# yl602019618/Reconstruction-of-PDE-without-Time-Label

Measured on AMD Instinct MI355X. Metric: snapshot-bags/sec (train step) + rel-L2 drift error, 2D FPE 128² @1/2/4/8 GPU, higher is better.
Workload: dtype f32; 1 GPU; 2d_FPE train_fno.py NIOFP2D_FNO(2,3,100,25,3,12,32,2) (C), grid 128x128; per_gpu_batch=4, global_batch=4, T=100, bag_size=L=randint(50,T) with replacement, dataset_bags=4096, parallelism=dp1, optimizer=Adam lr 0.0005 (fused flat), launch=hip-graph per bag size L (all kernels replayed each step)

## Files before the change

### include/blindno.h

```cpp
#ifndef BLINDNO_H
#define BLINDNO_H

#include <stdint.h>

#ifdef __cplusplus
extern "C" {
#endif

typedef void* blindno_stream_t;

int blindno_abi_version(void);
const char* blindno_error_string(int code);


int blindno_lift_fwd(const float* in, const float* w0, const float* b0, float* x0,
                     int Bn, int N1, int N2, int Cin, int C, int P1, int P2,
                     blindno_stream_t stream);

int blindno_lift_bwd(const float* dx0, const float* in, const float* w0, float* d_in,
                     float* partial, int nchunk,
                     int Bn, int N1, int N2, int Cin, int C, int P1, int P2,
                     blindno_stream_t stream);
int blindno_lift_bwd_nchunk(int Bn, int N1, int N2);

int blindno_project_fwd(const float* z, const float* w1, const float* b1, const float* w2,
                        const float* b2, float* out, int Bn, int C, int P1, int P2, int Ho,
                        int Wo, int Hd, int Cout, int ostride, int ooff,
                        blindno_stream_t stream);

int blindno_project_bwd(const float* z, const float* w1, const float* b1, const float* w2,
                        const float* dout, float* dz, float* partial, int nchunk,
                        int Bn, int C, int P1, int P2, int Ho, int Wo, int Hd, int Cout,
                        int ostride, int ooff, int dout_div, blindno_stream_t stream);
int blindno_project_bwd_nchunk(int Bn, int Ho, int Wo);
int blindno_project_bwd_nchunk_heads(int Bg, int Ho, int Wo);
int blindno_project_bwd_w(const float* z, const float* w1, const float* b1, const float* w2,
                          const float* dout, const float* lscale, float* dz, float* partial,
                          int nchunk, int Bn, int C, int P1, int P2, int Ho, int Wo, int Hd,
                          int Cout, int ostride, int ooff, int dout_div, blindno_stream_t stream);

int64_t blindno_project_bag_stats_floats(int B, int Ho, int Wo);
int blindno_project_bag_bwd_nchunk(int B, int Ho, int Wo);
int blindno_project_bag_fwd(const float* z, const float* w1, const float* b1, const float* w2,
                            const float* b2, const float* lw, float* ubar, float* stats,
                            float* v, int B, int U, int C, int P1, int P2, int Ho, int Wo, int Hd,
                            blindno_stream_t stream);
int blindno_project_bag_bwd(const float* stats, const float* gs, const float* w2, const float* lw,
                            const float* v, float* dz, float* partial, int nchunk, int B, int U,
                            int C, int P1, int P2, int Ho, int Wo, int Hd,
                            blindno_stream_t stream);


int blindno_rowdft(const float* x, float* At, const float* Tp, int Bn, int C, int P1,
                   int P2, int m2, int act, blindno_stream_t stream);
int blindno_rowdft_crop(const float* x, float* At, const float* Tp, int Bn, int C, int P1,
                        int P2, int m2, int act, int N1v, int N2v, blindno_stream_t stream);

int blindno_colpass(const float* At, const float* Wt, float* Xs, float* Y, float* Z,
                    const float* FB, const float* GB, int Bn, int Ci, int Co, int P1, int m1,
                    int m2, int P2, int dir, blindno_stream_t stream);

int blindno_mix_wgrad_nsplit(int Bn, int Ci, int Co, int K1, int m2);
int blindno_mix_wgrad(const float* X, const float* G, float* dWt, float* partial, int nsplit,
                      int Bn, int Ci, int Co, int K1, int m2, blindno_stream_t stream);
int blindno_mix_wgrad_part(const float* X, const float* G, float* partial, int nsplit, int Gw,
                           int Bn, int Ci, int Co, int K1, int m2, blindno_stream_t stream);
int blindno_mix_wgrad_multi(const void* const* X, const void* const* G, void* const* out,
                            const int* shp, int njobs, blindno_stream_t stream);
int blindno_mix_wgrad_multi_u(const void* const* X, const void* const* G, void* const* out,
                              const int* shp, void* const* ud, const int* um1, int njobs,
                              blindno_stream_t stream);

int blindno_mix1d(const float* At, const float* Wt, float* Xs, float* Z, int Bn, int Ci,
                  int Co, int m, int P2, int dir, blindno_stream_t stream);

int blindno_rowidft_epi(const float* Z, const float* x, const float* wc, const float* bc,
                        float* z, const float* tb, int Bn, int C, int P1, int P2, int m2,
                        int act, blindno_stream_t stream);
int blindno_rowidft_epi_crop(const float* Z, const float* x, const float* wc, const float* bc,
// ... 385 lines not shown
```

### reconstruction-of-pde-without-time-label_amd/blindno/_lib.py

```python
from __future__ import annotations

import ctypes
import os
import threading

import torch

_HERE = os.path.dirname(os.path.abspath(__file__))
LIB_PATH = os.environ.get("BLINDNO_LIB", os.path.join(_HERE, "libblindno.so"))

SIGNATURES = {
    "blindno_abi_version": "",
    "blindno_lift_fwd": "ppppiiiiiiis",
    "blindno_lift_bwd": "pppppiiiiiiiis",
    "blindno_project_fwd": "ppppppiiiiiiiiiis",
    "blindno_project_bwd": "pppppppiiiiiiiiiiiis",
    "blindno_rowdft": "pppiiiiiis",
    "blindno_rowdft_crop": "pppiiiiiiiis",
    "blindno_rowdft_bag_lift": "ppppppiiiiiiiiis",
    "blindno_rowdft_bag_lift_dg": "pppppppiiiiiiiiis",
    "blindno_rowidft_epi_lift": "ppppppppppiiiiiiiiis",
    "blindno_rowidft_bwd_lift": "ppppppppppiiiiiiiiis",
    "blindno_colpass": "pppppppiiiiiiiis",
    "blindno_colspec_ok": "iiiiii",
# ... 36 lines not shown
    "blindno_mse_fwd": "ppplipppps",
    "blindno_rowsq": "pppiiiiiis",
    "blindno_adam": "pppplddffffs",
    "blindno_gpe_solve": "ppppddiiipppiiis",
    "blindno_trapz_rows": "ppppiis",
    "blindno_lift_bwd_nchunk": "iii",
    "blindno_conv_wgrad_nchunk": "iii",
    "blindno_rowidft_bwd_nchunk": "iiiii",
    "blindno_set_rowfuse": "i",
    "blindno_set_colfuse": "i",
    "blindno_project_bwd_nchunk": "iii",
    "blindno_project_bwd_nchunk_heads": "iii",
    "blindno_mix_wgrad_nsplit": "iiiii",
    "blindno_lift_fwd_g": "ppppiliiiiiiis",
    "blindno_lift_fwd_bag_g": "ppppiliiiiiiippppfs",
    "blindno_lift_bag_ok": "iiiiiiii",
    "blindno_lift_bwd_g": "pppppiiliiiiiiis",
    "blindno_lift_bwd_mix_g": "pppppiiliiiiiiippppiiis",
    "blindno_lift_bwd_bag_mix_g": "pppppiiliiiiiiippppiiippppffs",
    "blindno_project_fwd_g": "ppppppiliiiiiiiiiis",
    "blindno_project_bwd_g": "pppppppiiliiiiiiiiiis",
    "blindno_colpass_g": "pppppppiliiiiiiiis",
    "blindno_mix_wgrad_g": "ppppiiiiiiis",
    "blindno_rowidft_epi_g": "ppppppiliiiiiis",
    "blindno_rowidft_bwd_g": "ppppppiliiiiiis",
    "blindno_conv_wgrad_g": "pppiiiiiiis",
    "blindno_rowdft_wgrad_ok": "iiiii",
    "blindno_rowdft_wgrad_g": "pppppiippppiiiiiiiis",
    "blindno_bagmean_fwd_w": "pppppp" + "iiiii" + "s",
    "blindno_project_bwd_w": "pppppppp" + "i" + "iiiiiiiiiii" + "s",
    "blindno_project_bag_stats_floats": "iii",
    "blindno_project_bag_bwd_nchunk": "iii",
    "blindno_project_bag_fwd": "ppppppppp" + "iiiiiiii" + "s",
    "blindno_project_bag_bwd": "ppppppp" + "i" + "iiiiiiii" + "s",
    "blindno_pack_w2d_2": "ppppp" + "iiiii" + "s",
    "blindno_unpack_w2d_2": "ppppp" + "iiiii" + "s",
    "blindno_bn_act_nslices": "iii",
    "blindno_bn_act_fwd": "ppppppppiiiifffis",
    "blindno_bn_act_bwd": "pppppppppiiiifis",
    "blindno_gather_flat": "pppips",
    "blindno_gather_batch": "ppppipis",
    "blindno_reduce_partials_multi": "ppppis",
    "blindno_reduce_partials_pieces": "ppppppis",
    "blindno_reduce_partials_pieces_u": "pppppppppis",
    "blindno_reduce_segs_limit": "i",
    "blindno_finish_multi": "pppppppppippppis",
    "blindno_unpack_w2d_multi": "ppppis",
    "blindno_pack_w2d_multi": "ppppis",
    "blindno_fp_propagate": "pppiiiiiids",
    "blindno_bagattn_nchunk": "i",
    "blindno_bagattn_fwd": "pppppppp" + "iiii" + "s",
    "blindno_bagattn_bwd": "ppppppppppp" + "iiii" + "s",
    "blindno_conv2d_fwd": "pppp" + "iiiiiiiiiii" + "s",
    "blindno_conv2d_bwd_data": "ppp" + "iiiiiiiiiii" + "s",
    "blindno_conv2d_wgrad_nsplit": "iiiiiiiiiii",
    "blindno_conv2d_bwd_weight": "pppp" + "i" + "iiiiiiiiiii" + "s",
    "blindno_conv2d_fwd_nsplit": "iiiiiiiiiii",
    "blindno_conv2d_fwd_split": "ppppp" + "i" + "p" + "iiiiiiiiiii" + "s",
    "blindno_conv2d_bwd_data_nsplit": "iiiiiiiiiii",
    "blindno_conv2d_bwd_data_split": "pppp" + "i" + "p" + "iiiiiiiiiii" + "s",
    "blindno_conv2d_wscratch_floats": "i" + "iiiiiiiiiii",
    "blindno_spectral2d_tables_bytes": "iiii",
    "blindno_spectral2d_tables_init": "piiii",
    "blindno_spectral_conv2d_workspace_bytes": "iiiiiiii",
    "blindno_spectral_conv2d_saved_bytes": "iiiii",
    "blindno_spectral_conv2d_fwd": "ppppppp" + "iiiiiii" + "s",
# ... 129 lines not shown
```

### reconstruction-of-pde-without-time-label_amd/blindno/ops.py

```python
from __future__ import annotations

import contextlib
import ctypes
import math
from typing import List, Optional, Sequence, Tuple

import torch

from ._lib import BlindnoError, call, ptr, query, stream_ptr

F32 = torch.float32

MIX_F16 = False

BAG_STATS = True
BAG_STATS_MAX_BYTES = 4 << 30

COLSPEC = True
HEAD_BWD_MERGED = True
UNPACK_FOLD = True
HOST_ENC_MIX = True
HOST_PACK = True


def set_mix_precision(name: str) -> None:
    global MIX_F16
    if name not in ("fp32", "fp16"):
        raise BlindnoError(f"mix precision must be 'fp32' or 'fp16', got {name!r}")
    MIX_F16 = name == "fp16"


def _mixdir(direction: int) -> int:
    return direction | (2 if MIX_F16 else 0)



def pad_amount(n: int) -> int:
    return int(round(n * 0.25))


def kept_rows_count(m1: int, P1: int) -> int:
    return 2 * m1 if 2 * m1 < P1 else P1


_TW = {}


def twiddle(P: int, device) -> torch.Tensor:
    dev = torch.device(device)
# ... 1373 lines not shown
         ptr(twiddle_colspec(P1, m1, grid.device)), 1, 3, P1, P2, m2, 0, P1, P2, stream_ptr())
    K1 = kept_rows_count(m1, P1)
    Dg2 = _empty(1, m2, 3, K1, 2, like=grid)
    call("blindno_colmix", ptr(part), nb, None, ptr(Dg2), None, 1, 3, 3, P1, P2, m1, m2, 0, None, None,
         None, stream_ptr())
    if not capturing:
        if len(_DG2_CACHE) > 16:
            _DG2_CACHE.clear()
        _DG2_CACHE[key] = (grid, Dg2)
    return Dg2


class _ColSpec:

    def __init__(self, Bn, C, P1, P2, m1, m2, device):
        self.Bn, self.C, self.P1, self.P2, self.m1, self.m2 = Bn, C, P1, P2, m1, m2
        self.K1 = kept_rows_count(m1, P1)
        self.nb = P1 // 16
        self.tab = twiddle_colspec(P1, m1, device)
        self.Tp = twiddle_mfma(P2, m2, device)
        self.tb = twiddle_rowinv(P2, m2, device)

    def part(self, Cp, like):
        return _empty(self.Bn * self.nb * query("blindno_colspec_nchunk", Cp, self.m2) * 128, like=like)

    def mix(self, part, nbv, Wt, direction, Cp=None, lift=None):
        Xs = _empty(self.Bn, self.m2, self.C, self.K1, 2, like=part)
        Y = _empty(self.Bn, self.m2, self.C, self.K1, 2, like=part)
        w0, b0, Dg2 = lift if lift is not None else (None, None, None)
        call("blindno_colmix", ptr(part), nbv, ptr(Wt), ptr(Xs), ptr(Y), self.Bn, self.C,
             Cp or self.C, self.P1, self.P2, self.m1, self.m2, direction, ptr(w0), ptr(b0), ptr(Dg2),
             stream_ptr())
        return Xs, Y


def _bag_stats_ok(B, L, C, P1, P2, Ho, Wo, Hd, Cout):
    if not (BAG_STATS and Hd == 128 and Cout == 1 and L <= 1024):
        return False
    nstats = query("blindno_project_bag_stats_floats", B, Ho, Wo)
    return 4 * (nstats + B * L * C * P1 * P2) <= BAG_STATS_MAX_BYTES


def bag_ubar_ok(meta, B, L, N1, N2, fc1w, fc2w, head_meta, G, width):
    fake = (B * L, N1, N2, 3)
    _, _, _, _, P1, P2, Ho, Wo = _fno_geometry(fake, meta)
    if not _bag_stats_ok(B, L, meta.width, P1, P2, Ho, Wo, fc1w.shape[0], fc2w.shape[0]):
        return False
    hP1, hP2 = _fno_geometry((B, N1, N2, width), head_meta)[4:6]
    return query("blindno_lift_bag_ok", G, G * B, N1, N2, width, head_meta.width, hP1, hP2) == 1


class BagHeadsIn:

    def __init__(self, grid, bw, bb):
        self.grid, self.w, self.b = _c(grid), _c(bw.detach()), _c(bb.detach())
        self.width = bw.shape[0]

    def shape(self, ubar):
        return (ubar.shape[0], ubar.shape[1], ubar.shape[2], self.width)


class BagEncoderFn(torch.autograd.Function):

    @staticmethod
    def forward(ctx, meta, emit_ubar, X, idx_t, lw, grid, bw, bb, *prm):
        require_device(X, grid, *prm)
# ... 65 lines not shown
                tb = ptr(twiddle_rowinv(P2, meta.m2, X.device))
                if last:
                    call("blindno_rowidft_epi_lift", ptr(Z), ptr(X), ptr(idx_t), ptr(grid), ptr(fc0w),
                         ptr(fc0b), ptr(cw), ptr(cb), ptr(z), tb, B, T, L, N1, N2, C, P1, P2,
                         meta.m2, stream_ptr())
                else:
                    At_next = _empty(Bn, meta.m2, C, P1, 2, like=X)
                    call("blindno_rowidft_epi_lift_rd", ptr(Z), ptr(X), ptr(idx_t), ptr(grid),
                         ptr(fc0w), ptr(fc0b), ptr(cw), ptr(cb), ptr(z), tb, B, T, L, N1, N2, C, P1,
                         P2, meta.m2, ptr(At_next), ptr(twiddle_mfma(P2, meta.m2, X.device)), 1,
                         stream_ptr())
            else:
                Xk, Z = spec_forward(zs[-1], 1, Wt, sh, At=At_next)
                if last:
                    z = _empty(Bn, C, P1, P2, like=X)
                    call("blindno_rowidft_epi_crop", ptr(Z), ptr(zs[-1]), ptr(cw), ptr(cb), ptr(z),
                         ptr(twiddle_rowinv(P2, meta.m2, X.device)), Bn, C, P1, P2, meta.m2, 1, Ho, Wo,
                         stream_ptr())
                else:
                    z, At_next = k_rowidft_epi_rd(Z, zs[-1], cw, cb, Bn, C, P1, P2, meta.m2, 1, 1)
            Xs.append(Xk)
            Wts.append(Wt)
            zs.append(z)
        fc1w, fc1b, fc2w, fc2b = prm[2 + 4 * n:6 + 4 * n]
        Hd, Cout = fc1w.shape[0], fc2w.shape[0]
        S = Ho * Wo
        width = bw.shape[0]
        h = _empty(B, S, width, like=X)
        ctx.bag = None
        if _bag_stats_ok(B, L, C, P1, P2, Ho, Wo, Hd, Cout):
            ubar = _empty(B, S, like=X)
            stats = _empty(query("blindno_project_bag_stats_floats", B, Ho, Wo), like=X)
            v = _empty(Bn, C, P1, P2, like=X)
            call("blindno_project_bag_fwd", ptr(zs[-1]), ptr(fc1w), ptr(fc1b), ptr(fc2w), ptr(fc2b),
                 ptr(lw), ptr(ubar), ptr(stats), ptr(v), B, L, C, P1, P2, Ho, Wo, Hd, stream_ptr())
            if not emit_ubar:
                call("blindno_bagmean_fwd_w", ptr(ubar), ptr(grid), ptr(bw), ptr(bb), None, ptr(h), B, 1,
                     S, 2, width, stream_ptr())
            ctx.bag = (stats, v)
        elif emit_ubar:
            raise BlindnoError("BagEncoderFn: emit_ubar needs the bag-level projection (bag_ubar_ok)")
        else:
            u = _empty(Bn, Ho, Wo, Cout, like=X)
            call("blindno_project_fwd", ptr(zs[-1]), ptr(fc1w), ptr(fc1b), ptr(fc2w), ptr(fc2b), ptr(u),
                 Bn, C, P1, P2, Ho, Wo, Hd, Cout, Cout, 0, stream_ptr())
            call("blindno_bagmean_fwd_w", ptr(u), ptr(grid), ptr(bw), ptr(bb), ptr(lw), ptr(h), B, L, S,
                 2, width, stream_ptr())
        ctx.meta, ctx.n, ctx.dims = meta, n, (B, T, L, N1, N2, C, P1, P2, Ho, Wo, Hd, Cout, width)
        ctx.lw = lw
        ctx.emit_ubar = bool(emit_ubar)
        ctx.save_for_backward(X, idx_t, grid, bw, *Xs, *Wts, *zs, *prm)
        if emit_ubar:
            return ubar.view(B, N1, N2)
        return h.view(B, N1, N2, width)

    @staticmethod
    def backward(ctx, gh):
        meta, n = ctx.meta, ctx.n
        B, T, L, N1, N2, C, P1, P2, Ho, Wo, Hd, Cout, width = ctx.dims
        t = ctx.saved_tensors
        X, idx_t, grid, bw = t[:4]
        Xs, Wts, zs = list(t[4:4 + n]), list(t[4 + n:4 + 2 * n]), list(t[4 + 2 * n:4 + 3 * n])
        prm = list(t[4 + 3 * n:])
        Bn, S = B * L, Ho * Wo
        gh = _c(gh)
        grads = [None] * len(prm)
        lw = ctx.lw
        bag = ctx.bag
# ... 510 lines not shown
```

### reconstruction-of-pde-without-time-label_amd/blindno/timing.py

```python
from __future__ import annotations

import os

import torch

from . import _lib

GELU_FLOPS = 0
DOMINANT = os.environ.get("BLINDNO_TIMED_KERNEL", "blindno_project_bag_fwd")
_VARIANTS = {"blindno_project_bwd": ("blindno_project_bwd", "blindno_project_bwd_w"),
             "blindno_conv2d": ("blindno_conv2d_fwd", "blindno_conv2d_bwd_data", "blindno_conv2d_bwd_weight",
                                "blindno_conv2d_fwd_split", "blindno_conv2d_bwd_data_split")}
_CONV_ARG0 = {"blindno_conv2d_fwd": 4, "blindno_conv2d_bwd_data": 3, "blindno_conv2d_bwd_weight": 5,
              "blindno_conv2d_fwd_split": 7, "blindno_conv2d_bwd_data_split": 6}
_FAMILIES = ("blindno_conv2d",)


def _conv_out(n, k, s, p):
    return (n + 2 * p - k) // s + 1


def _i(args, k):
    return int(args[k])


def _present(a):
    return a is not None and getattr(a, "value", a) is not None


def cost(name, args):
    if name == "blindno_rowdft":
        Bn, C, P1, P2, m2 = (_i(args, k) for k in range(3, 8))
        return 4 * Bn * C * P1 * P2 + 8 * Bn * m2 * C * P1, 4 * Bn * C * P1 * P2 * m2
    if name == "blindno_rowidft_epi":
        has_wc = _present(args[2])
        Bn, C, P1, P2, m2 = (_i(args, k) for k in range(6, 11))
        pts = Bn * C * P1 * P2
        return 8 * Bn * C * P1 * m2 + 4 * pts * (2 if has_wc else 1), pts * (4 * m2 + (2 * C if has_wc else 0))
    if name == "blindno_rowidft_bwd":
        has_wc, act = _present(args[2]), _i(args, 11)
        Bn, C, P1, P2, m2 = (_i(args, k) for k in range(6, 11))
        pts = Bn * C * P1 * P2
        return (8 * Bn * C * P1 * m2 + 4 * pts * (2 + int(has_wc) + int(act > 0)),
                pts * (4 * m2 + (2 * C if has_wc else 0)))
    if name == "blindno_project_fwd":
        Bn, C, P1, P2, Ho, Wo, Hd, Cout = (_i(args, k) for k in range(6, 14))
        pts = Bn * Ho * Wo
        return 4 * pts * (C + Cout), pts * Hd * (2 * C + 2 * Cout + GELU_FLOPS)
    if name in ("blindno_project_bwd", "blindno_project_bwd_w"):
        o = 8 if name == "blindno_project_bwd" else 9
        Bn, C, P1, P2, Ho, Wo, Hd, Cout = (_i(args, k) for k in range(o, o + 8))
        dout_div = _i(args, o + 10)
        pts = Bn * Ho * Wo
        return (8 * pts * C + 4 * (pts // max(1, dout_div)) * Cout,
                pts * Hd * (6 * C + 4 * Cout + 1 + 2 * GELU_FLOPS))
    if name == "blindno_project_bag_fwd":
        B, U, C, P1, P2, Ho, Wo, Hd = (_i(args, k) for k in range(9, 17))
        pts, bpts = B * U * Ho * Wo, B * Ho * Wo
        return (8 * pts * C + 4 * ((bpts + 15) // 16) * 16 * Hd * 6 + 4 * bpts,
                pts * Hd * (6 * C + 4 + 2 * GELU_FLOPS))
    if name == "blindno_project_bag_bwd":
        B, U, C, P1, P2, Ho, Wo, Hd = (_i(args, k) for k in range(8, 16))
        pts, bpts = B * U * Ho * Wo, B * Ho * Wo
        return 8 * pts * C + 4 * ((bpts + 15) // 16) * 16 * Hd * 6 + 4 * bpts, 2 * bpts * Hd * 6
    if name in _CONV_ARG0:
        o = _CONV_ARG0[name]
        N, Ci, Hi, Wi, Co, KH, KW, sh, sw, ph, pw = (_i(args, k) for k in range(o, o + 11))
        Ho, Wo = _conv_out(Hi, KH, sh, ph), _conv_out(Wi, KW, sw, pw)
        K = Ci * KH * KW + (1 if name == "blindno_conv2d_bwd_weight" else 0)
        flops = 2 * N * Co * Ho * Wo * K
        nbytes = 4 * (N * Ci * Hi * Wi + N * Co * Ho * Wo + Co * K)
        return nbytes, flops
    if name == "blindno_colpass3d":
        Bn, Ci, Co, P1, P2, P3, m1, m2, m3, d = (_i(args, k) for k in range(7, 17))
        cin, cout = (Ci, Co) if d == 0 else (Co, Ci)
        K1, K2 = min(2 * m1, P1), min(2 * m2, P2)
        nbytes = 8 * (Bn * m3 * (cin + cout) * P1 * P2 + Bn * m3 * cin * K1 * K2 + m3 * K1 * K2 * Ci * Co)
        flops = 8 * Bn * m3 * ((cin + cout) * (P1 * P2 * K2 + P1 * K2 * K1) + K1 * K2 * Ci * Co)
        return nbytes, flops
    if name == "blindno_conv_wgrad":
        nchunk, Bn, C, P1, P2 = (_i(args, k) for k in range(3, 8))
        pts = Bn * P1 * P2
        return 8 * C * pts, 2 * pts * (C * C + C)
    return 0, 0


def pmc_record(root: str, name: str):
    import json
    p = os.path.join(root, "profiles", "pmc_traffic.json")
    if not os.path.exists(p):
        return None
    return json.load(open(p)).get(name)


def pmc_traffic(root: str, name: str):
    import json
    p = os.path.join(root, "profiles", "pmc_traffic.json")
    if not os.path.exists(p):
        return None
    d = json.load(open(p)).get(name)
    return None if d is None else float(d["bytes_per_point"])


def points(name, args):
    if name == "blindno_project_bag_fwd":
        return _i(args, 9) * _i(args, 10) * _i(args, 14) * _i(args, 15)
    if name in ("blindno_project_bwd", "blindno_project_bwd_w", "blindno_project_fwd"):
        o = {"blindno_project_bwd": 8, "blindno_project_bwd_w": 9, "blindno_project_fwd": 6}[name]
        Bn, Ho, Wo = _i(args, o), _i(args, o + 4), _i(args, o + 5)
        return Bn * Ho * Wo
    return 0


class KernelTimer:

    def __init__(self, name: str = DOMINANT):
        self.name = name
        self.entries = _VARIANTS.get(name, (name,))
        self.recs = []
        self._pending = None

    class _Hook:
        def __init__(self, timer, entry):
            self.timer, self.entry = timer, entry

        def before(self, args):
            ev = torch.cuda.Event(enable_timing=True)
            ev.record()
            self.timer._pending = ev

        def after(self, args):
            ev = torch.cuda.Event(enable_timing=True)
            ev.record()
            b, f = cost(self.entry, args)
            self.timer.recs.append((self.timer._pending, ev, b, f, points(self.entry, args)))

    def start(self):
        for e in self.entries:
# ... 45 lines not shown
```

### reconstruction-of-pde-without-time-label_amd/build.py

```python
#!/usr/bin/env python3
from __future__ import annotations

import argparse
import concurrent.futures as cf
import glob
import os
import shutil
import subprocess
import sys

HERE = os.path.dirname(os.path.abspath(__file__))
CSRC = os.path.join(HERE, "csrc")
OUT = os.path.join(HERE, "blindno", "libblindno.so")
BUILD = os.path.join(HERE, "build")
INCLUDE = os.path.join(os.path.dirname(HERE), "include")
ARCH = os.environ.get("BLINDNO_ARCH", "gfx950")

CXXFLAGS = ["-O3", "-fPIC", "-std=c++17", f"--offload-arch={ARCH}", "-I", INCLUDE, "-I", CSRC,
            "-fvisibility=hidden", "-Wall", "-Wno-unused-function", "-Wno-unused-result"]


FILE_FLAGS = {"project.hip": ["-fno-slp-vectorize", "-mllvm", "-amdgpu-mfma-vgpr-form"],
              "bagproj.hip": ["-fno-slp-vectorize", "-mllvm", "-amdgpu-mfma-vgpr-form"]}


def _hipcc():
    h = shutil.which("hipcc") or "/opt/rocm/bin/hipcc"
    if not os.path.exists(h):
        raise RuntimeError("hipcc not found (ROCm toolchain required to build libblindno)")
    return h


def _newer(src_list, dst):
    if not os.path.exists(dst):
        return True
    t = os.path.getmtime(dst)
    return any(os.path.getmtime(s) > t for s in src_list)


def build(force: bool = False, jobs: int = 8, verbose: bool = True) -> str:
    hipcc = _hipcc()
    os.makedirs(BUILD, exist_ok=True)
    srcs = sorted(glob.glob(os.path.join(CSRC, "*.hip")))
    headers = glob.glob(os.path.join(CSRC, "*.h")) + glob.glob(os.path.join(INCLUDE, "*.h"))
    objs = []
    todo = []
    for s in srcs:
        o = os.path.join(BUILD, os.path.basename(s)[:-4] + ".o")
        objs.append(o)
        if force or _newer([s] + headers, o):
            todo.append((s, o))

    def compile_one(so):
        s, o = so
        cmd = [hipcc, *CXXFLAGS, *FILE_FLAGS.get(os.path.basename(s), []), "-c", s, "-o", o]
        r = subprocess.run(cmd, capture_output=True, text=True)
# ... 48 lines not shown
```

### reconstruction-of-pde-without-time-label_amd/csrc/bagproj.hip

```cpp
#include "common.h"
#include "blindno.h"
#include "gelu_pk.h"

using namespace blindno;
using namespace blindno::gelu_pk;

namespace {

typedef float f32x4 __attribute__((ext_vector_type(4)));

constexpr int kHd = 128;
constexpr int kNStat = 6;
constexpr int kTileF4 = (kHd / 16) * kNStat * 64;
constexpr int kMaxU = 1024;
#ifndef BAGPROJ_QUAD
#define BAGPROJ_QUAD 1
#endif
#ifndef BAGPROJ_FWD_WAVES
#define BAGPROJ_FWD_WAVES 3
#endif
#ifndef BAGPROJ_SETUP2
#define BAGPROJ_SETUP2 1
#endif

// ... 11 lines not shown
#define BAGPROJ_BWD_UNROLL 1
#endif
#ifndef BAGPROJ_SC
#define BAGPROJ_SC 8
#endif
constexpr int kSC2 = BAGPROJ_SC;

__device__ __forceinline__ float swap_sum32(float a, float b) {
  const auto r = __builtin_amdgcn_permlane32_swap(__float_as_uint(a), __float_as_uint(b), false, false);
  return __uint_as_float(r[0]) + __uint_as_float(r[1]);
}

__device__ __forceinline__ float swap_sum16(float a, float b) {
  const auto r = __builtin_amdgcn_permlane16_swap(__float_as_uint(a), __float_as_uint(b), false, false);
  return __uint_as_float(r[0]) + __uint_as_float(r[1]);
}

#ifndef BAGPROJ_PROBE
#define BAGPROJ_PROBE 0
#endif
#if BAGPROJ_PROBE
__device__ unsigned long long g_bagproj_probe[32768 * 8];
#define BP_MARK(i)                                                                          \
  do {                                                                                      \
    __builtin_amdgcn_sched_barrier(0);                                                      \
    const unsigned long long t_ = __builtin_amdgcn_s_memrealtime();                         \
    const int slot_ = blockIdx.x * 4 + (threadIdx.x >> 6);                                  \
    if ((threadIdx.x & 63) == 0 && slot_ < 32768) g_bagproj_probe[slot_ * 8 + (i)] = t_;    \
    __builtin_amdgcn_sched_barrier(0);                                                      \
  } while (0)
#else
#define BP_MARK(i) do {} while (0)
#endif
__global__ __launch_bounds__(256, BAGPROJ_FWD_WAVES) void bagproj_fwd_kernel(
    const float* __restrict__ z, const float* __restrict__ w1, const float* __restrict__ b1,
    const float* __restrict__ w2, const float* __restrict__ b2, const float* __restrict__ lw,
    float* __restrict__ ubar, float* __restrict__ stats, float* __restrict__ v, BagGeom g) {
  __shared__ float slw[kMaxU];
  __shared__ float zs[2][kSC2][16][4];
  __shared__ float zw[2][kSC2][16][4];
  __shared__ float vred[2][4][kSC2][64];
  __shared__ float zbr[4][64];
  __shared__ float vpart[16][4];
  __shared__ float vhalf[4];
  __shared__ float ured[4][16];
  __shared__ float2 swr[4][4][2][2][4];
  const int tid = threadIdx.x, lane = tid & 63;
  const int wave = uniform_int(tid >> 6);
  const int c16 = lane & 15, g4 = lane >> 4;
  const int C = (int)g.C, U = (int)g.U;
  BP_MARK(0);
  const int cs = (tid >> 4) & 3, ls = tid >> 6;
  const unsigned ntiles = (g.npts + 15) / 16;
  auto zload = [&](unsigned bo, bool ok, int ch, float (&zr)[kSC2 / 4]) {
#pragma unroll
    for (int i = 0; i < kSC2 / 4; ++i) {
      const int lg = ch * kSC2 + ls + 4 * i;
#if BAGPROJ_SETUP2
      const int lc = lg < U ? lg : U - 1, cc = cs < C ? cs : C - 1;
      const float zv = z[bo + (unsigned)(lc * C + cc) * g.HW];
      zr[i] = (ok && lg < U && cs < C) ? zv : 0.f;
#else
      zr[i] = (ok && lg < U && cs < C) ? z[bo + (unsigned)(lg * C + cs) * g.HW] : 0.f;
#endif
    }
  };
  float wa[2], bb[2][4], vloc[4] = {0.f, 0.f, 0.f, 0.f};
#if BAGPROJ_SETUP2
  __shared__ float sw1[kHd * 4], sb1[kHd], sw2[kHd];
  constexpr int kLwIt = kMaxU / 256;
  float lwv[kLwIt], w1v[2], b1v = 0.f, w2v = 0.f;
#pragma unroll
  for (int i = 0; i < kLwIt; ++i) {
    const int l = tid + 256 * i;
    lwv[i] = l < U ? (lw ? lw[l] : 1.0f / (float)U) : 0.f;
  }
#pragma unroll
  for (int i = 0; i < 2; ++i) w1v[i] = tid + 256 * i < kHd * C ? w1[tid + 256 * i] : 0.f;
  if (tid < kHd) {
    b1v = b1[tid];
    w2v = w2[tid];
  }
  float zfirst[kSC2 / 4];
  {
    const unsigned f = blockIdx.x * 16 + (unsigned)c16;
    const bool ok = f < g.npts;
    zload(g.base(ok ? f : 0u), ok, 0, zfirst);
  }
#pragma unroll
  for (int i = 0; i < kLwIt; ++i)
    if (tid + 256 * i < U) slw[tid + 256 * i] = lwv[i];
#pragma unroll
  for (int i = 0; i < 2; ++i)
    if (tid + 256 * i < kHd * C) sw1[tid + 256 * i] = w1v[i];
// ... 32 lines not shown
    for (int r = 0; r < 4; ++r) {
      const int k = k0 + 4 * g4 + r;
      bb[tt][r] = kK * b1[k];
      if (c16 == 0) {
#pragma unroll
        for (int c = 0; c < 4; ++c) {
          const float wrv = c < C ? w2[k] * w1[k * C + c] : 0.f;
          vloc[c] += wrv;
          float2& e = swr[wave][g4][tt][r >> 1][c];
          if (r & 1) e.y = wrv; else e.x = wrv;
        }
      }
    }
  }
#endif
  if (c16 == 0) {
#pragma unroll
    for (int c = 0; c < 4; ++c) vpart[4 * wave + g4][c] = 0.5f * vloc[c];
  }
  __syncthreads();
  if (tid < 4) {
    float acc = 0.f;
    for (int j = 0; j < 16; ++j) acc += vpart[j][tid];
    vhalf[tid] = acc;
  }
#if !BAGPROJ_SETUP2
  float lsum = 0.f;
  for (int l = 0; l < U; ++l) lsum += slw[l];
  const float b2l = b2[0] * lsum;
#endif
  BP_MARK(1);

  const int nch = (U + kSC2 - 1) / kSC2;
  for (unsigned tile = blockIdx.x; tile < ntiles; tile += gridDim.x) {
    const unsigned f = tile * 16 + (unsigned)c16;
    const bool ok = f < g.npts;
    const unsigned bo = g.base(ok ? f : 0u);
    float zbp = 0.f;
    float zn[kSC2 / 4];
    auto load = [&](int ch) { zload(bo, ok, ch, zn); };
    auto store = [&](int ch, int buf) {
#pragma unroll
      for (int i = 0; i < kSC2 / 4; ++i) {
        const int l = ls + 4 * i, lg = ch * kSC2 + l;
        const float wv = zn[i] * slw[lg < U ? lg : 0];
        zs[buf][l][c16][cs] = zn[i];
        zw[buf][l][c16][cs] = wv;
        zbp += wv;
      }
    };
    auto vwrite = [&](int ch, int buf) {
#pragma unroll
      for (int i = 0; i < kSC2 / 4; ++i) {
        const int l = ls + 4 * i, lg = ch * kSC2 + l;
        if (ok && lg < U && cs < C)
          v[bo + (unsigned)(lg * C + cs) * g.HW] =
              (((vred[buf][0][l][lane] + vred[buf][1][l][lane]) + vred[buf][2][l][lane]) +
               vred[buf][3][l][lane]) + vhalf[cs];
      }
    };
    f32x2 A[2][2], S[2][2], Q[2][4][2];
#pragma unroll
    for (int tt = 0; tt < 2; ++tt)
#pragma unroll
      for (int i = 0; i < 2; ++i) {
        A[tt][i] = S[tt][i] = (f32x2){0.f, 0.f};
#pragma unroll
        for (int c = 0; c < 4; ++c) Q[tt][c][i] = (f32x2){0.f, 0.f};
      }
    if (BAGPROJ_SETUP2 && tile == blockIdx.x) {
#pragma unroll
      for (int i = 0; i < kSC2 / 4; ++i) zn[i] = zfirst[i];
    } else {
      load(0);
    }
    store(0, 0);
    if (nch > 1) load(1);
#if BAGPROJ_SETUP2
    float lsum = 0.f;
#endif
    __syncthreads();
    BP_MARK(2);
    for (int ch = 0; ch < nch; ++ch) {
      const int buf = ch & 1, l0 = ch * kSC2;
      const int nl = U - l0 < kSC2 ? U - l0 : kSC2;
      for (int l = 0; l < nl; ++l) {
        int zo;
        asm volatile("v_mov_b32 %0, 0" : "=v"(zo));
        const float4 zc = *reinterpret_cast<const float4*>(&zw[buf][l][c16][0]);
        const float az = zs[buf][l][c16][g4];
        const float lwl = slw[l0 + l];
        const f32x2 wl = splat2(lwl);
#if BAGPROJ_SETUP2
        lsum += lwl;
#endif
        f32x2 vp[4];
#if BAGPROJ_QUAD
        f32x2 hq[4], sq[4], eq[4];
#pragma unroll
        for (int tt = 0; tt < 2; ++tt) {
          f32x4 d = {bb[tt][0], bb[tt][1], bb[tt][2], bb[tt][3]};
          d = __builtin_amdgcn_mfma_f32_16x16x4f32(wa[tt], az, d, 0, 0, 0);
          hq[2 * tt] = (f32x2){d[0], d[1]};
          hq[2 * tt + 1] = (f32x2){d[2], d[3]};
        }
        norm_cdf_quad_pdf_centered(hq, sq, eq);
#endif
#pragma unroll
        for (int tt = 0; tt < 2; ++tt) {
#if !BAGPROJ_QUAD
          f32x4 d = {bb[tt][0], bb[tt][1], bb[tt][2], bb[tt][3]};
          d = __builtin_amdgcn_mfma_f32_16x16x4f32(wa[tt], az, d, 0, 0, 0);
          const f32x2 h[2] = {{d[0], d[1]}, {d[2], d[3]}};
#else
          const f32x2 h[2] = {hq[2 * tt], hq[2 * tt + 1]};
#endif
#pragma unroll
          for (int i = 0; i < 2; ++i) {
#if BAGPROJ_QUAD
            const f32x2 ep = eq[2 * tt + i], sg = sq[2 * tt + i];
#else
            f32x2 ep;
            const f32x2 sg = norm_cdf_pair_pdf_centered(h[i], ep);
#endif
            const f32x2 gd = pk_fma(h[i], ep, sg);
            A[tt][i] = pk_fma(wl, h[i] * sg, A[tt][i]);
            S[tt][i] = pk_fma(wl, gd, S[tt][i]);
            Q[tt][0][i] = pk_fma(gd, splat2(zc.x), Q[tt][0][i]);
            Q[tt][1][i] = pk_fma(gd, splat2(zc.y), Q[tt][1][i]);
            Q[tt][2][i] = pk_fma(gd, splat2(zc.z), Q[tt][2][i]);
            Q[tt][3][i] = pk_fma(gd, splat2(zc.w), Q[tt][3][i]);
            const float4* wq = reinterpret_cast<const float4*>(&swr[wave][g4][tt][i][0]) + zo;
            const float4 wq0 = wq[0], wq1 = wq[1];
            const f32x2 q0 = {wq0.x, wq0.y}, q1 = {wq0.z, wq0.w}, q2 = {wq1.x, wq1.y}, q3 = {wq1.z, wq1.w};
            if (tt == 0 && i == 0) {
              vp[0] = gd * q0; vp[1] = gd * q1; vp[2] = gd * q2; vp[3] = gd * q3;
            } else {
              vp[0] = pk_fma(gd, q0, vp[0]);
              vp[1] = pk_fma(gd, q1, vp[1]);
              vp[2] = pk_fma(gd, q2, vp[2]);
              vp[3] = pk_fma(gd, q3, vp[3]);
            }
          }
        }
        const float a = swap_sum32(vp[0].x + vp[0].y, vp[2].x + vp[2].y);
        const float b = swap_sum32(vp[1].x + vp[1].y, vp[3].x + vp[3].y);
        vred[buf][wave][l][lane] = swap_sum16(a, b);
      }
      if (ch + 1 < nch) {
        store(ch + 1, buf ^ 1);
        if (ch + 2 < nch) load(ch + 2);
      }
      if (ch >= 1) vwrite(ch - 1, buf ^ 1);
      __syncthreads();
    }
    vwrite(nch - 1, (nch - 1) & 1);
#if BAGPROJ_SETUP2
    const float b2l = b2[0] * lsum;
#endif
    zbr[ls][lane] = zbp;
    BP_MARK(3);
    __syncthreads();
    float4* st = reinterpret_cast<float4*>(stats) + (size_t)tile * kTileF4 + lane;
    float zb[4];
#pragma unroll
    for (int c = 0; c < 4; ++c)
      zb[c] = ((zbr[0][16 * c + c16] + zbr[1][16 * c + c16]) + zbr[2][16 * c + c16]) + zbr[3][16 * c + c16];
    float up = 0.f;
#pragma unroll
    for (int tt = 0; tt < 2; ++tt) {
      const int t = 2 * wave + tt;
      float av[4];
#pragma unroll
      for (int r = 0; r < 4; ++r) {
        const int k = 16 * t + 4 * g4 + r;
#if BAGPROJ_SETUP2
        float hb = sb1[k] * lsum;
#pragma unroll
        for (int c = 0; c < 4; ++c) hb = c < C ? fmaf(sw1[k * C + c], zb[c], hb) : hb;
#else
        float hb = b1[k] * lsum;
#pragma unroll
        for (int c = 0; c < 4; ++c) hb = c < C ? fmaf(w1[k * C + c], zb[c], hb) : hb;
#endif
        const float acc = r == 0 ? A[tt][0].x : (r == 1 ? A[tt][0].y : (r == 2 ? A[tt][1].x : A[tt][1].y));
        av[r] = fmaf(kInvK, acc, 0.5f * hb);
      }
      const float4 a4 = {av[0], av[1], av[2], av[3]};
      const int kb = 16 * t + 4 * g4;
#if BAGPROJ_SETUP2
      up += (sw2[kb] * a4.x + sw2[kb + 1] * a4.y) + (sw2[kb + 2] * a4.z + sw2[kb + 3] * a4.w);
#else
      up += (w2[kb] * a4.x + w2[kb + 1] * a4.y) + (w2[kb + 2] * a4.z + w2[kb + 3] * a4.w);
#endif
      st[(t * kNStat + 0) * 64] = a4;
      const float hs = 0.5f * lsum;
      st[(t * kNStat + 1) * 64] = (float4){S[tt][0].x + hs, S[tt][0].y + hs, S[tt][1].x + hs, S[tt][1].y + hs};
#pragma unroll
      for (int c = 0; c < 4; ++c) {
        const float hz = 0.5f * zb[c];
        st[(t * kNStat + 2 + c) * 64] =
            (float4){Q[tt][c][0].x + hz, Q[tt][c][0].y + hz, Q[tt][c][1].x + hz, Q[tt][c][1].y + hz};
      }
    }
    up += __shfl_xor(up, 16, 64);
    up += __shfl_xor(up, 32, 64);
    if (g4 == 0) ured[wave][c16] = up;
    __syncthreads();
    if (tid < 16 && ok) ubar[f] = (((ured[0][tid] + ured[1][tid]) + ured[2][tid]) + ured[3][tid]) + b2l;
  }
  BP_MARK(4);
#if BAGPROJ_PROBE
  if ((threadIdx.x & 63) == 0) {
    const int slot_ = blockIdx.x * 4 + (threadIdx.x >> 6);
    if (slot_ < 32768) {
      g_bagproj_probe[slot_ * 8 + 5] = __builtin_amdgcn_s_getreg((31 << 11) | 4);
      g_bagproj_probe[slot_ * 8 + 6] = __builtin_amdgcn_s_getreg((31 << 11) | 20);
    }
  }
#endif
}
#if BAGPROJ_PROBE
BLINDNO_API int blindno_bagproj_probe_read(unsigned long long* dst, int n) {
  return (int)hipMemcpyFromSymbol(dst, HIP_SYMBOL(g_bagproj_probe),
                                  sizeof(unsigned long long) * (size_t)n, 0, hipMemcpyDeviceToHost);
}
#endif

__global__ __launch_bounds__(256) void bagproj_bwd_kernel(
    const float* __restrict__ stats, const float* __restrict__ gs, const float* __restrict__ w2,
    const float* __restrict__ lw, const float* __restrict__ v, float* __restrict__ dz,
    float* __restrict__ partial, BagGeom g) {
  constexpr int kJ = kTileF4 / 256;
  __shared__ float slw[kMaxU];
  __shared__ float4 red[kJ * 4][4];
  __shared__ float sgs;
  const int tid = threadIdx.x, lane = tid & 63, c16 = lane & 15;
  const int C = (int)g.C, U = (int)g.U;
  for (int l = tid; l < U; l += 256) slw[l] = lw ? lw[l] : 1.0f / (float)U;
  __syncthreads();
  float4 acc[kJ];
#pragma unroll
// ... 87 lines not shown
}

bool bag_geom(int B, int U, int C, int P1, int P2, int Ho, int Wo, int Hd, BagGeom& g) {
  if (B < 1 || U < 1 || U > kMaxU || C < 1 || C > 4 || Hd != kHd || Ho < 1 || Wo < 1 || Ho > P1 ||
      Wo > P2)
    return false;
  if ((int64_t)B * U * C * P1 * P2 >= INT32_MAX || (int64_t)B * Ho * Wo >= INT32_MAX) return false;
  g.npts = (unsigned)(B * Ho * Wo);
  g.S = (unsigned)(Ho * Wo);
  g.Wo = (unsigned)Wo;
  g.P2 = (unsigned)P2;
  g.HW = (unsigned)(P1 * P2);
  g.C = (unsigned)C;
  g.U = (unsigned)U;
  g.dS = FastDiv::make(g.S);
  g.dWo = FastDiv::make(g.Wo);
  return true;
}

}

BLINDNO_API int64_t blindno_project_bag_stats_floats(int B, int Ho, int Wo) {
  return ((int64_t)B * Ho * Wo + 15) / 16 * (int64_t)kTileF4 * 4;
}

#ifndef BAGPROJ_BWD_BLOCKS
#define BAGPROJ_BWD_BLOCKS 1024
#endif
BLINDNO_API int blindno_project_bag_bwd_nchunk(int B, int Ho, int Wo) {
  const int64_t tiles = ((int64_t)B * Ho * Wo + 15) / 16;
  return (int)(tiles < 1 ? 1 : (tiles > BAGPROJ_BWD_BLOCKS ? BAGPROJ_BWD_BLOCKS : tiles));
}

BLINDNO_API int blindno_project_bag_fwd(const float* z, const float* w1, const float* b1,
                                        const float* w2, const float* b2, const float* lw,
                                        float* ubar, float* stats, float* v, int B, int U, int C,
                                        int P1, int P2, int Ho, int Wo, int Hd, void* stream) {
  BagGeom g;
  if (!bag_geom(B, U, C, P1, P2, Ho, Wo, Hd, g) || !z || !ubar || !stats || !v)
    return (int)hipErrorInvalidValue;
  const unsigned ntiles = (g.npts + 15) / 16;
  bagproj_fwd_kernel<<<ntiles, 256, 0, (hipStream_t)stream>>>(z, w1, b1, w2, b2, lw, ubar, stats,
                                                               v, g);
  return (int)hipGetLastError();
}

BLINDNO_API int blindno_project_bag_bwd(const float* stats, const float* gs, const float* w2,
                                        const float* lw, const float* v, float* dz,
                                        float* partial, int nchunk, int B, int U, int C, int P1,
                                        int P2, int Ho, int Wo, int Hd, void* stream) {
  BagGeom g;
  if (!bag_geom(B, U, C, P1, P2, Ho, Wo, Hd, g) || !stats || !gs || (dz && !v) || !partial ||
      nchunk < 1)
    return (int)hipErrorInvalidValue;
  bagproj_bwd_kernel<<<nchunk, 256, 0, (hipStream_t)stream>>>(stats, gs, w2, lw, v, dz, partial, g);
  return (int)hipGetLastError();
}
```

Baseline: 3662 snapshot-bags/s.

## Make bag projection forward a persistent kernel with atomic tile scheduling

Adds a persistent-grid variant of the bag projection forward kernel. It launches one workgroup per occupancy slot, and workgroups draw tiles dynamically from a global atomic counter. Each workgroup prefetches the first z chunk of its next tile during the last chunk of the current one, and the address math is simplified to clamped unsigned offsets. The goal is to cut per-workgroup launch and setup cost and the tail imbalance. In exchange it adds atomics, a self-resetting counter that must stay consistent across graph replays, and a new compile flag that disables the atomic optimizer.

```diff
diff --git a/include/blindno.h b/include/blindno.h
--- a/include/blindno.h
+++ b/include/blindno.h
@@ -45,6 +45,11 @@
                             const float* b2, const float* lw, float* ubar, float* stats,
                             float* v, int B, int U, int C, int P1, int P2, int Ho, int Wo, int Hd,
                             blindno_stream_t stream);
+int blindno_project_bag_fwd_grid(int B, int Ho, int Wo, int nwg);
+int blindno_project_bag_fwd_p(const float* z, const float* w1, const float* b1, const float* w2,
+                              const float* b2, const float* lw, float* ubar, float* stats,
+                              float* v, int B, int U, int C, int P1, int P2, int Ho, int Wo,
+                              int Hd, int* counters, int nwg, blindno_stream_t stream);
 int blindno_project_bag_bwd(const float* stats, const float* gs, const float* w2, const float* lw,
                             const float* v, float* dz, float* partial, int nchunk, int B, int U,
                             int C, int P1, int P2, int Ho, int Wo, int Hd,
diff --git a/reconstruction-of-pde-without-time-label_amd/blindno/_lib.py b/reconstruction-of-pde-without-time-label_amd/blindno/_lib.py
--- a/reconstruction-of-pde-without-time-label_amd/blindno/_lib.py
+++ b/reconstruction-of-pde-without-time-label_amd/blindno/_lib.py
@@ -92,6 +92,8 @@
     "blindno_project_bag_stats_floats": "iii",
     "blindno_project_bag_bwd_nchunk": "iii",
     "blindno_project_bag_fwd": "ppppppppp" + "iiiiiiii" + "s",
+    "blindno_project_bag_fwd_grid": "iiii",
+    "blindno_project_bag_fwd_p": "ppppppppp" + "iiiiiiii" + "pi" + "s",
     "blindno_project_bag_bwd": "ppppppp" + "i" + "iiiiiiii" + "s",
     "blindno_pack_w2d_2": "ppppp" + "iiiii" + "s",
     "blindno_unpack_w2d_2": "ppppp" + "iiiii" + "s",
diff --git a/reconstruction-of-pde-without-time-label_amd/blindno/ops.py b/reconstruction-of-pde-without-time-label_amd/blindno/ops.py
--- a/reconstruction-of-pde-without-time-label_amd/blindno/ops.py
+++ b/reconstruction-of-pde-without-time-label_amd/blindno/ops.py
@@ -15,6 +15,7 @@
 
 BAG_STATS = True
 BAG_STATS_MAX_BYTES = 4 << 30
+BAGPROJ_PERSIST = True
 
 COLSPEC = True
 HEAD_BWD_MERGED = True
@@ -1454,6 +1455,20 @@
              Cp or self.C, self.P1, self.P2, self.m1, self.m2, direction, ptr(w0), ptr(b0), ptr(Dg2),
              stream_ptr())
         return Xs, Y
+
+
+_BAG_COUNTERS = {}
+
+
+def bag_counters(grid, device):
+    key = (int(grid), str(device))
+    t = _BAG_COUNTERS.get(key)
+    if t is None:
+        t = torch.zeros(2, dtype=torch.int32, device=device)
+        t[:1].fill_(int(grid))
+        if not torch.cuda.is_current_stream_capturing():
+            _BAG_COUNTERS[key] = t
+    return t
 
 
 def _bag_stats_ok(B, L, C, P1, P2, Ho, Wo, Hd, Cout):
@@ -1585,8 +1600,14 @@
             ubar = _empty(B, S, like=X)
             stats = _empty(query("blindno_project_bag_stats_floats", B, Ho, Wo), like=X)
             v = _empty(Bn, C, P1, P2, like=X)
-            call("blindno_project_bag_fwd", ptr(zs[-1]), ptr(fc1w), ptr(fc1b), ptr(fc2w), ptr(fc2b),
-                 ptr(lw), ptr(ubar), ptr(stats), ptr(v), B, L, C, P1, P2, Ho, Wo, Hd, stream_ptr())
+            if BAGPROJ_PERSIST:
+                ctr = bag_counters(query("blindno_project_bag_fwd_grid", B, Ho, Wo, 0), X.device)
+                call("blindno_project_bag_fwd_p", ptr(zs[-1]), ptr(fc1w), ptr(fc1b), ptr(fc2w), ptr(fc2b),
+                     ptr(lw), ptr(ubar), ptr(stats), ptr(v), B, L, C, P1, P2, Ho, Wo, Hd, ptr(ctr), 0,
+                     stream_ptr())
+            else:
+                call("blindno_project_bag_fwd", ptr(zs[-1]), ptr(fc1w), ptr(fc1b), ptr(fc2w), ptr(fc2b),
+                     ptr(lw), ptr(ubar), ptr(stats), ptr(v), B, L, C, P1, P2, Ho, Wo, Hd, stream_ptr())
             if not emit_ubar:
                 call("blindno_bagmean_fwd_w", ptr(ubar), ptr(grid), ptr(bw), ptr(bb), None, ptr(h), B, 1,
                      S, 2, width, stream_ptr())
diff --git a/reconstruction-of-pde-without-time-label_amd/blindno/timing.py b/reconstruction-of-pde-without-time-label_amd/blindno/timing.py
--- a/reconstruction-of-pde-without-time-label_amd/blindno/timing.py
+++ b/reconstruction-of-pde-without-time-label_amd/blindno/timing.py
@@ -9,6 +9,7 @@
 GELU_FLOPS = 0
 DOMINANT = os.environ.get("BLINDNO_TIMED_KERNEL", "blindno_project_bag_fwd")
 _VARIANTS = {"blindno_project_bwd": ("blindno_project_bwd", "blindno_project_bwd_w"),
+             "blindno_project_bag_fwd": ("blindno_project_bag_fwd", "blindno_project_bag_fwd_p"),
              "blindno_conv2d": ("blindno_conv2d_fwd", "blindno_conv2d_bwd_data", "blindno_conv2d_bwd_weight",
                                 "blindno_conv2d_fwd_split", "blindno_conv2d_bwd_data_split")}
 _CONV_ARG0 = {"blindno_conv2d_fwd": 4, "blindno_conv2d_bwd_data": 3, "blindno_conv2d_bwd_weight": 5,
@@ -54,7 +55,7 @@
         pts = Bn * Ho * Wo
         return (8 * pts * C + 4 * (pts // max(1, dout_div)) * Cout,
                 pts * Hd * (6 * C + 4 * Cout + 1 + 2 * GELU_FLOPS))
-    if name == "blindno_project_bag_fwd":
+    if name in ("blindno_project_bag_fwd", "blindno_project_bag_fwd_p"):
         B, U, C, P1, P2, Ho, Wo, Hd = (_i(args, k) for k in range(9, 17))
         pts, bpts = B * U * Ho * Wo, B * Ho * Wo
         return (8 * pts * C + 4 * ((bpts + 15) // 16) * 16 * Hd * 6 + 4 * bpts,
@@ -103,7 +104,7 @@
 
 
 def points(name, args):
-    if name == "blindno_project_bag_fwd":
+    if name in ("blindno_project_bag_fwd", "blindno_project_bag_fwd_p"):
         return _i(args, 9) * _i(args, 10) * _i(args, 14) * _i(args, 15)
     if name in ("blindno_project_bwd", "blindno_project_bwd_w", "blindno_project_fwd"):
         o = {"blindno_project_bwd": 8, "blindno_project_bwd_w": 9, "blindno_project_fwd": 6}[name]
diff --git a/reconstruction-of-pde-without-time-label_amd/build.py b/reconstruction-of-pde-without-time-label_amd/build.py
--- a/reconstruction-of-pde-without-time-label_amd/build.py
+++ b/reconstruction-of-pde-without-time-label_amd/build.py
@@ -21,7 +21,8 @@
 
 
 FILE_FLAGS = {"project.hip": ["-fno-slp-vectorize", "-mllvm", "-amdgpu-mfma-vgpr-form"],
-              "bagproj.hip": ["-fno-slp-vectorize", "-mllvm", "-amdgpu-mfma-vgpr-form"]}
+              "bagproj.hip": ["-fno-slp-vectorize", "-mllvm", "-amdgpu-mfma-vgpr-form",
+                              "-mllvm", "-amdgpu-atomic-optimizer-strategy=None"]}
 
 
 def _hipcc():
diff --git a/reconstruction-of-pde-without-time-label_amd/csrc/bagproj.hip b/reconstruction-of-pde-without-time-label_amd/csrc/bagproj.hip
--- a/reconstruction-of-pde-without-time-label_amd/csrc/bagproj.hip
+++ b/reconstruction-of-pde-without-time-label_amd/csrc/bagproj.hip
@@ -67,10 +67,14 @@
 #else
 #define BP_MARK(i) do {} while (0)
 #endif
+template <bool kPersist>
 __global__ __launch_bounds__(256, BAGPROJ_FWD_WAVES) void bagproj_fwd_kernel(
     const float* __restrict__ z, const float* __restrict__ w1, const float* __restrict__ b1,
     const float* __restrict__ w2, const float* __restrict__ b2, const float* __restrict__ lw,
-    float* __restrict__ ubar, float* __restrict__ stats, float* __restrict__ v, BagGeom g) {
+    float* __restrict__ ubar, float* __restrict__ stats, float* __restrict__ v, BagGeom g,
+    unsigned* __restrict__ counters) {
+  static_assert(!kPersist || BAGPROJ_SETUP2, "the persistent grid carries zfirst across tiles");
+  __shared__ unsigned snext;
   __shared__ float slw[kMaxU];
   __shared__ float zs[2][kSC2][16][4];
   __shared__ float zw[2][kSC2][16][4];
@@ -87,14 +91,18 @@
   BP_MARK(0);
   const int cs = (tid >> 4) & 3, ls = tid >> 6;
   const unsigned ntiles = (g.npts + 15) / 16;
+  const unsigned chw = g.C * g.HW, lsofs = (unsigned)ls * chw, csofs = (unsigned)cs * g.HW;
+  const unsigned cstep = (unsigned)kSC2 * chw, istep = 4u * chw;
+  const unsigned lastofs = (g.U - 1) * chw, ccofs = (unsigned)(cs < C ? cs : C - 1) * g.HW;
   auto zload = [&](unsigned bo, bool ok, int ch, float (&zr)[kSC2 / 4]) {
 #pragma unroll
     for (int i = 0; i < kSC2 / 4; ++i) {
       const int lg = ch * kSC2 + ls + 4 * i;
 #if BAGPROJ_SETUP2
-      const int lc = lg < U ? lg : U - 1, cc = cs < C ? cs : C - 1;
-      const float zv = z[bo + (unsigned)(lc * C + cc) * g.HW];
-      zr[i] = (ok && lg < U && cs < C) ? zv : 0.f;
+      const unsigned lo = lsofs + (unsigned)ch * cstep + (unsigned)i * istep;
+      zr[i] = z[bo + ccofs + (lo < lastofs ? lo : lastofs)];
+      (void)ok;
+      (void)lg;
 #else
       zr[i] = (ok && lg < U && cs < C) ? z[bo + (unsigned)(lg * C + cs) * g.HW] : 0.f;
 #endif
@@ -193,7 +201,8 @@
   BP_MARK(1);
 
   const int nch = (U + kSC2 - 1) / kSC2;
-  for (unsigned tile = blockIdx.x; tile < ntiles; tile += gridDim.x) {
+  for (unsigned tile = blockIdx.x; tile < ntiles;) {
+    unsigned tnext = tile + gridDim.x, tdrawn = 0;
     const unsigned f = tile * 16 + (unsigned)c16;
     const bool ok = f < g.npts;
     const unsigned bo = g.base(ok ? f : 0u);
@@ -204,8 +213,9 @@
 #pragma unroll
       for (int i = 0; i < kSC2 / 4; ++i) {
         const int l = ls + 4 * i, lg = ch * kSC2 + l;
-        const float wv = zn[i] * slw[lg < U ? lg : 0];
-        zs[buf][l][c16][cs] = zn[i];
+        const float zv = (ok && lg < U && cs < C) ? zn[i] : 0.f;
+        const float wv = zv * slw[lg < U ? lg : 0];
+        zs[buf][l][c16][cs] = zv;
         zw[buf][l][c16][cs] = wv;
         zbp += wv;
       }
@@ -215,7 +225,7 @@
       for (int i = 0; i < kSC2 / 4; ++i) {
         const int l = ls + 4 * i, lg = ch * kSC2 + l;
         if (ok && lg < U && cs < C)
-          v[bo + (unsigned)(lg * C + cs) * g.HW] =
+          v[bo + csofs + lsofs + (unsigned)ch * cstep + (unsigned)i * istep] =
               (((vred[buf][0][l][lane] + vred[buf][1][l][lane]) + vred[buf][2][l][lane]) +
                vred[buf][3][l][lane]) + vhalf[cs];
       }
@@ -229,14 +239,23 @@
 #pragma unroll
         for (int c = 0; c < 4; ++c) Q[tt][c][i] = (f32x2){0.f, 0.f};
       }
-    if (BAGPROJ_SETUP2 && tile == blockIdx.x) {
+    if (kPersist || (BAGPROJ_SETUP2 && tile == blockIdx.x)) {
 #pragma unroll
       for (int i = 0; i < kSC2 / 4; ++i) zn[i] = zfirst[i];
     } else {
       load(0);
     }
+    auto prefetch = [&]() {
+      tnext = (unsigned)uniform_int((int)snext);
+      const unsigned fn = tnext * 16 + (unsigned)c16;
+      const bool okn = tnext < ntiles && fn < g.npts;
+      zload(g.base(okn ? fn : 0u), okn, 0, zfirst);
+    };
     store(0, 0);
     if (nch > 1) load(1);
+    if constexpr (kPersist) {
+      if (tid == 0) tdrawn = __hip_atomic_fetch_add(counters, 1u, __ATOMIC_RELAXED, __HIP_MEMORY_SCOPE_AGENT);
+    }
 #if BAGPROJ_SETUP2
     float lsum = 0.f;
 #endif
@@ -245,6 +264,9 @@
     for (int ch = 0; ch < nch; ++ch) {
       const int buf = ch & 1, l0 = ch * kSC2;
       const int nl = U - l0 < kSC2 ? U - l0 : kSC2;
+      if constexpr (kPersist) {
+        if (ch >= 1 && ch == nch - 1) prefetch();
+      }
       for (int l = 0; l < nl; ++l) {
         int zo;
         asm volatile("v_mov_b32 %0, 0" : "=v"(zo));
@@ -308,12 +330,18 @@
         const float b = swap_sum32(vp[1].x + vp[1].y, vp[3].x + vp[3].y);
         vred[buf][wave][l][lane] = swap_sum16(a, b);
       }
+      if constexpr (kPersist) {
+        if (ch == 0 && tid == 0) snext = tdrawn;
+      }
       if (ch + 1 < nch) {
         store(ch + 1, buf ^ 1);
         if (ch + 2 < nch) load(ch + 2);
       }
       if (ch >= 1) vwrite(ch - 1, buf ^ 1);
       __syncthreads();
+    }
+    if constexpr (kPersist) {
+      if (nch == 1) prefetch();
     }
     vwrite(nch - 1, (nch - 1) & 1);
 #if BAGPROJ_SETUP2
@@ -369,6 +397,18 @@
     if (g4 == 0) ured[wave][c16] = up;
     __syncthreads();
     if (tid < 16 && ok) ubar[f] = (((ured[0][tid] + ured[1][tid]) + ured[2][tid]) + ured[3][tid]) + b2l;
+    tile = tnext;
+  }
+  if constexpr (kPersist) {
+    if (tid == 0) {
+      const unsigned arrived =
+          __hip_atomic_fetch_add(counters + 1, 1u, __ATOMIC_RELAXED, __HIP_MEMORY_SCOPE_AGENT);
+      if (arrived == gridDim.x - 1) {
+        __hip_atomic_store(counters, gridDim.x, __ATOMIC_RELAXED, __HIP_MEMORY_SCOPE_AGENT);
+        __hip_atomic_store(counters + 1, 0u, __ATOMIC_RELAXED, __HIP_MEMORY_SCOPE_AGENT);
+        __threadfence();
+      }
+    }
   }
   BP_MARK(4);
 #if BAGPROJ_PROBE
@@ -522,17 +562,57 @@
   return (int)(tiles < 1 ? 1 : (tiles > BAGPROJ_BWD_BLOCKS ? BAGPROJ_BWD_BLOCKS : tiles));
 }
 
+static int bagproj_fwd_slots() {
+  constexpr int kMaxDev = 64;
+  static int cached[kMaxDev];
+  int dev = 0, cus = 0;
+  if (hipGetDevice(&dev) != hipSuccess) return 0;
+  if (dev >= 0 && dev < kMaxDev && cached[dev] > 0) return cached[dev];
+  if (hipDeviceGetAttribute(&cus, hipDeviceAttributeMultiprocessorCount, dev) != hipSuccess || cus < 1)
+    return 0;
+  const int slots = cus * BAGPROJ_FWD_WAVES;
+  if (dev >= 0 && dev < kMaxDev) cached[dev] = slots;
+  return slots;
+}
+
+static int bagproj_fwd_grid(int64_t ntiles, int nwg) {
+  if (ntiles < 1 || nwg < 0) return 0;
+  const int64_t want = nwg > 0 ? nwg : bagproj_fwd_slots();
+  return (int)(want < ntiles ? want : ntiles);
+}
+
+BLINDNO_API int blindno_project_bag_fwd_grid(int B, int Ho, int Wo, int nwg) {
+  if (B < 1 || Ho < 1 || Wo < 1 || (int64_t)B * Ho * Wo >= INT32_MAX) return 0;
+  return bagproj_fwd_grid(((int64_t)B * Ho * Wo + 15) / 16, nwg);
+}
+
+BLINDNO_API int blindno_project_bag_fwd_p(const float* z, const float* w1, const float* b1,
+                                          const float* w2, const float* b2, const float* lw,
+                                          float* ubar, float* stats, float* v, int B, int U, int C,
+                                          int P1, int P2, int Ho, int Wo, int Hd, int* counters,
+                                          int nwg, void* stream) {
+  BagGeom g;
+  if (!bag_geom(B, U, C, P1, P2, Ho, Wo, Hd, g) || !z || !ubar || !stats || !v || nwg < 0)
+    return (int)hipErrorInvalidValue;
+  const unsigned ntiles = (g.npts + 15) / 16;
+  if (!counters) {
+    bagproj_fwd_kernel<false><<<ntiles, 256, 0, (hipStream_t)stream>>>(z, w1, b1, w2, b2, lw, ubar,
+                                                                        stats, v, g, nullptr);
+    return (int)hipGetLastError();
+  }
+  const int grid = bagproj_fwd_grid(ntiles, nwg);
+  if (grid < 1) return (int)hipErrorInvalidValue;
+  bagproj_fwd_kernel<true><<<grid, 256, 0, (hipStream_t)stream>>>(
+      z, w1, b1, w2, b2, lw, ubar, stats, v, g, reinterpret_cast<unsigned*>(counters));
+  return (int)hipGetLastError();
+}
+
 BLINDNO_API int blindno_project_bag_fwd(const float* z, const float* w1, const float* b1,
                                         const float* w2, const float* b2, const float* lw,
                                         float* ubar, float* stats, float* v, int B, int U, int C,
                                         int P1, int P2, int Ho, int Wo, int Hd, void* stream) {
-  BagGeom g;
-  if (!bag_geom(B, U, C, P1, P2, Ho, Wo, Hd, g) || !z || !ubar || !stats || !v)
-    return (int)hipErrorInvalidValue;
-  const unsigned ntiles = (g.npts + 15) / 16;
-  bagproj_fwd_kernel<<<ntiles, 256, 0, (hipStream_t)stream>>>(z, w1, b1, w2, b2, lw, ubar, stats,
-                                                               v, g);
-  return (int)hipGetLastError();
+  return blindno_project_bag_fwd_p(z, w1, b1, w2, b2, lw, ubar, stats, v, B, U, C, P1, P2, Ho, Wo, Hd,
+                                   nullptr, 0, stream);
 }
 
 BLINDNO_API int blindno_project_bag_bwd(const float* stats, const float* gs, const float* w2,
```

After: 3694 snapshot-bags/s, median of 6. Within noise of the previous version (+0.9%).
